# christoskokas/gtsam-vSLAM

Hardware: AMD Instinct MI355X
Metric: frames/sec (extract+match+localBA), 1500 feat stereo 752x480 (higher is better)
Workload: dtype u8/i32 (extract, match) + f64 (pose LM, local BA)

## Files before the change

### gtsam-vslam_amd/csrc/newpts.hip

```cpp
#include "proj_dev.hpp"
#include "track_dev.hpp"
#include "dmath.hpp"
#include <vector>
#include <mutex>

namespace vslam {

constexpr int NP_MAX_KF = 16;
constexpr int NP_MAX_ROWS = 4 * NP_MAX_KF;

struct NpKf {
    DPose Twc, Tcw;
    const vslam_keypoint* kpsL; const vslam_keypoint* kpsR;
    const uint8_t* descL; const uint8_t* descR;
    const int* rightIdxs; const int* leftIdxs; const int* unF; const int* unFR;
    int nL, nR;
    int skip;
};
struct NpArgs {
    NpKf kf[NP_MAX_KF];
    int nKf;
    const float* depth; const uint8_t* hasMp; const double* mpXyz; const uint8_t* mpDesc;
    double fx, fy, cx, cy, b; int w, h;
    float scalePyr[MAX_LEVELS], sigma[MAX_LEVELS];
// ... 55 lines not shown
            uint4* dd = (uint4*)(A.cdesc + (size_t)pos * 32);
            dd[0] = s[0]; dd[1] = s[1];
        }
        run += tot;
    }
    if (threadIdx.x == 0) A.count[0] = run < A.cap ? run : A.cap;
}

__global__ __launch_bounds__(256) void k_np_match(const NpArgs* __restrict__ tab) {
    const NpArgs& A = *lane_entry(tab, blockIdx.z);
    const int lane = threadIdx.x & 63;
    const int wave = __builtin_amdgcn_readfirstlane(threadIdx.x >> 6);
    const int c = blockIdx.x * 4 + wave, k = blockIdx.y + 1;
    if (k >= A.nKf || c >= A.count[0]) return;
    const NpKf& K = A.kf[k];
    int outL = -2, outR = -2;
    if (K.skip) { if (lane == 0) { A.match[((size_t)c * NP_MAX_KF + k) * 2] = -2; A.match[((size_t)c * NP_MAX_KF + k) * 2 + 1] = -2; } return; }
    const double wp[3] = {A.wPos[3 * (size_t)c], A.wPos[3 * (size_t)c + 1], A.wPos[3 * (size_t)c + 2]};
    double p[3];
    mat3_vec(K.Tcw.R, wp, p);
    for (int q = 0; q < 3; q++) p[q] += K.Tcw.t[q];
    const double pRx3 = p[0] - A.b;
    bool hasL = false, hasR = false;
    float pLx = 0, pLy = 0, pRx = 0, pRy = 0;
    if (!(p[2] <= 0.0)) {
        const double invZ = 1.0f / p[2];
        const double u = A.fx * p[0] * invZ + A.cx, v = A.fy * p[1] * invZ + A.cy;
        const double uR = A.fx * pRx3 * invZ + A.cx, vR = A.fy * p[1] * invZ + A.cy;
        if (!(u < 15 || v < 15 || u >= A.w - 15 || v >= A.h - 15)) { hasL = true; pLx = (float)u; pLy = (float)v; }
        if (!(uR < 15 || vR < 15 || uR >= A.w - 15 || vR >= A.h - 15)) { hasR = true; pRx = (float)uR; pRy = (float)vR; }
    }
    const double d[3] = {wp[0] - K.Twc.t[0], wp[1] - K.Twc.t[1], wp[2] - K.Twc.t[2]};
    const float dist = (float)sqrt(d[0] * d[0] + d[1] * d[1] + d[2] * d[2]);
    const float dif = A.mds[c] / dist;
    const double qs = log((double)dif) / (double)A.logScale;
    int predScale = (int)qs;
    predScale += (predScale < qs);
    if (predScale < 0) predScale = 0; else if (predScale >= A.nLev) predScale = A.nLev - 1;
    uint32_t md[8];
    {
        const uint32_t* pd = (const uint32_t*)(A.cdesc + (size_t)c * 32);
#pragma unroll
        for (int q = 0; q < 8; q++) md[q] = pd[q];
    }
    __shared__ ProjArgs sS[4];
    ProjArgs& S = sS[threadIdx.x >> 6];
    S.Mdev = nullptr; S.gate = nullptr; S.gateMin = 0; S.mpv = nullptr; S.M = 0; S.rightIdxs = nullptr; S.leftIdxs = nullptr;
    S.kps[0] = K.kpsL; S.kps[1] = K.kpsR; S.desc[0] = K.descL; S.desc[1] = K.descR; S.n[0] = K.nL; S.n[1] = K.nR;
    S.rad = 4.f;
    S.cellStart[0] = S.cellStart[1] = nullptr; S.cellIdx[0] = S.cellIdx[1] = nullptr;
#pragma unroll
    for (int l = 0; l < MAX_LEVELS; l++) S.scalePyr[l] = A.scalePyr[l];
    S.xMult = A.xMult; S.yMult = A.yMult; S.xGrids = A.xGrids; S.yGrids = A.yGrids; S.mode = PROJ_STEREO;
    unsigned long long l2[2] = {KEY_NONE, KEY_NONE}, r2[2] = {KEY_NONE, KEY_NONE};
    if (hasL && pLx > 0 && pLy > 0) scan_side<2>(S, 0, md, pLx, pLy, predScale, K.unF, l2);
    if (hasR && pRx > 0 && pRy > 0) scan_side<2>(S, 1, md, pRx, pRy, predScale, K.unFR, r2);
    if (lane == 0) {
        const int matchDistLBA = 50;
        const float ratioLBA = 0.6f;
        const unsigned long long POS = KEY_POS_MASK;
        int bestDist = 256, bestIdx = -1, bestLev = -1, bestLev2 = -1, secDist = 256;
        if (l2[0] != KEY_NONE && key_dist(l2[0]) < 256) { bestDist = key_dist(l2[0]); bestIdx = key_idx(l2[0]); bestLev = key_oct(l2[0]); }
        if (l2[1] != KEY_NONE && key_dist(l2[1]) < 256 && bestIdx >= 0) {
            secDist = key_dist(l2[1]);
            bestLev2 = ((l2[1] & POS) > (l2[0] & POS)) ? bestLev : key_oct(l2[1]);
        }
        int bestDistR = 256, bestIdxR = -1, bestLevR = -1, bestLevR2 = -1, secDistR = 256;
        if (r2[0] != KEY_NONE && key_dist(r2[0]) < 256) { bestDistR = key_dist(r2[0]); bestIdxR = key_idx(r2[0]); bestLevR = key_oct(r2[0]); }
        if (r2[1] != KEY_NONE && key_dist(r2[1]) < 256 && bestIdxR >= 0) { secDistR = key_dist(r2[1]); bestLevR2 = key_oct(r2[1]); }
        bool right = false;
        if (bestDist > bestDistR) { bestDist = bestDistR; secDist = secDistR; bestLev = bestLevR; bestLev2 = bestLevR2; right = true; }
        bool ok = !(bestDist > matchDistLBA);
        if (ok && bestLev == bestLev2 && (float)bestDist >= ratioLBA * (float)secDist) ok = false;
        if (ok) {
            const int keyL = A.key[2 * c], keyR = A.key[2 * c + 1];
            const NpKf& K0 = A.kf[0];
            const vslam_keypoint kk = right ? (keyR >= 0 ? K0.kpsR[keyR] : K0.kpsL[keyL]) : (keyL >= 0 ? K0.kpsL[keyL] : K0.kpsR[keyR]);
            const double dx = (double)(right ? pRx : pLx) - (double)kk.x, dy = (double)(right ? pRy : pLy) - (double)kk.y;
            if (!(sqrt(dx * dx + dy * dy) > 10.0)) ok = false;
        }
        if (ok) {
            if (right) { outR = bestIdxR; const int l = K.leftIdxs[bestIdxR]; outL = l >= 0 ? l : -1; }
            else { outL = bestIdx; const int r = K.rightIdxs[bestIdx]; outR = r >= 0 ? r : -1; }
        }
        A.match[((size_t)c * NP_MAX_KF + k) * 2] = outL;
        A.match[((size_t)c * NP_MAX_KF + k) * 2 + 1] = outR;
    }
}

__device__ __forceinline__ bool np_dlt_point(double* sA, int t, int rows, double* pt) {
    auto a = [&](int r, int q) -> double& { return sA[((size_t)(r * 4 + q)) * 64 + t]; };
    if (rows < 4) return false;
    double V[16];
#pragma unroll
    for (int i = 0; i < 16; i++) V[i] = (i % 5 == 0) ? 1.0 : 0.0;
    for (int sweep = 0; sweep < 30; sweep++) {
        bool rotated = false;
#pragma unroll
        for (int p = 0; p < 3; p++)
#pragma unroll
            for (int q = p + 1; q < 4; q++) {
                double alpha = 0, beta = 0, gamma = 0;
                for (int r = 0; r < rows; r++) {
                    const double ap = a(r, p), aq = a(r, q);
                    alpha += ap * ap; beta += aq * aq; gamma += ap * aq;
                }
                if (gamma == 0.0 || fabs(gamma) <= 1e-15 * sqrt(alpha * beta)) continue;
                rotated = true;
                const double zeta = (beta - alpha) / (2.0 * gamma);
// ... 743 lines not shown
```

### gtsam-vslam_amd/csrc/proj.hip

```cpp
#include "matcher.hpp"
#include "proj_dev.hpp"
#include "track_dev.hpp"

namespace vslam {

__device__ __forceinline__ void load_mp_desc(const vslam_mappoint_view* mp, uint32_t (&md)[8]) {
    const uint32_t* p = (const uint32_t*)mp->desc;
#pragma unroll
    for (int k = 0; k < 8; k++) md[k] = p[k];
}

constexpr int PROJ_CELLS_NT = 1024;
__device__ __forceinline__ void proj_cells_body(const ProjArgs& A, int side) {
    extern __shared__ int cellHist[];
    __shared__ int wsum[PROJ_CELLS_NT / 64];
    const int tid = threadIdx.x, lane = tid & 63, wave = tid >> 6;
    int* cs = A.cellStart[side];
    unsigned short* ci = A.cellIdx[side];
    if (!cs || !ci) return;
    const int nCells = A.xGrids * A.yGrids, n = A.n[side];
    const vslam_keypoint* kps = A.kps[side];
    for (int c = tid; c < nCells; c += PROJ_CELLS_NT) cellHist[c] = 0;
    __syncthreads();
    for (int idx = tid; idx < n; idx += PROJ_CELLS_NT) {
        int cx = __float2int_rn(kps[idx].x * A.xMult), cy = __float2int_rn(kps[idx].y * A.yMult);
        cx = cx < 0 ? 0 : (cx >= A.xGrids ? A.xGrids - 1 : cx);
        cy = cy < 0 ? 0 : (cy >= A.yGrids ? A.yGrids - 1 : cy);
        atomicAdd(&cellHist[cy * A.xGrids + cx], 1);
    }
    __syncthreads();
    const int per = (nCells + PROJ_CELLS_NT - 1) / PROJ_CELLS_NT;
    const int c0 = min(tid * per, nCells), c1 = min(c0 + per, nCells);
    int mine = 0;
    for (int c = c0; c < c1; c++) mine += cellHist[c];
    int incl = mine;
#pragma unroll
    for (int d = 1; d < 64; d <<= 1) { const int t = __shfl_up(incl, d); if (lane >= d) incl += t; }
    if (lane == 63) wsum[wave] = incl;
    __syncthreads();
    int run = incl - mine;
    for (int k = 0; k < wave; k++) run += wsum[k];
    for (int c = c0; c < c1; c++) { const int v = cellHist[c]; cs[c] = run; cellHist[c] = run; run += v; }
    if (tid == PROJ_CELLS_NT - 1) cs[nCells] = run;
    __syncthreads();
    for (int idx = tid; idx < n; idx += PROJ_CELLS_NT) {
        int cx = __float2int_rn(kps[idx].x * A.xMult), cy = __float2int_rn(kps[idx].y * A.yMult);
        cx = cx < 0 ? 0 : (cx >= A.xGrids ? A.xGrids - 1 : cx);
        cy = cy < 0 ? 0 : (cy >= A.yGrids ? A.yGrids - 1 : cy);
        ci[atomicAdd(&cellHist[cy * A.xGrids + cx], 1)] = (unsigned short)idx;
    }
}
__global__ __launch_bounds__(PROJ_CELLS_NT) void k_proj_cells(ProjArgs A) { proj_cells_body(A, blockIdx.x); }
__global__ __launch_bounds__(PROJ_CELLS_NT) void k_proj_cells_b(const ProjLane* __restrict__ lanes) {
    const ProjLane& L = *lane_entry(lanes, blockIdx.y);
    proj_cells_body(L.A, blockIdx.x);
}
void launch_proj_cells(hipStream_t s, const ProjArgs& A) {
    if (!A.cellStart[0]) return;
    hipLaunchKernelGGL(k_proj_cells, dim3(A.mode == PROJ_STEREO ? 2 : 1), dim3(PROJ_CELLS_NT), (size_t)PROJ_MAX_CELLS * sizeof(int), s, A);
}

__device__ __forceinline__ void proj_candidates_body(const ProjArgs& A, const int* __restrict__ matches,
                                                     unsigned long long* __restrict__ topk,
                                                     unsigned long long* __restrict__ stats) {
    const int lane = threadIdx.x & 63;
    const int wave = __builtin_amdgcn_readfirstlane(threadIdx.x >> 6);
    const int job = blockIdx.x * 4 + wave;
    __shared__ unsigned int sTests;
    if (A.gate && *A.gate < A.gateMin) return;
    int M = A.M;
    if (A.Mdev) M = min(M, *A.Mdev);
    if (threadIdx.x == 0) sTests = 0;
    __syncthreads();
    int tests = 0;
    if (job < 2 * M) {
        const int i = job >> 1, side = job & 1;
        unsigned long long out[PROJ_K];
#pragma unroll
        for (int j = 0; j < PROJ_K; j++) out[j] = KEY_NONE;
        const vslam_mappoint_view* mp = A.mpv + i;
        const bool skip = matches[2 * i] >= 0 || matches[2 * i + 1] >= 0;
        const bool inF = side ? (A.mode == PROJ_STEREO && mp->in_frame_r) : mp->in_frame;
        if (!skip && inF) {
            uint32_t md[8];
            load_mp_desc(mp, md);
            const float px = side ? mp->pred_rx : mp->pred_lx, py = side ? mp->pred_ry : mp->pred_ly;
            const int ps = side ? mp->scale_level_r : mp->scale_level_l;
            tests = scan_side<PROJ_K>(A, side, md, px, py, ps, nullptr, out);
        }
        if (lane < PROJ_K) {
            unsigned long long v = out[0];
#pragma unroll
            for (int j = 1; j < PROJ_K; j++) v = lane == j ? out[j] : v;
            topk[(size_t)job * PROJ_K + lane] = v;
        }
    }
    if (lane == 0 && tests) atomicAdd(&sTests, (unsigned int)tests);
    __syncthreads();
    if (threadIdx.x == 0 && sTests) atomicAdd(&stats[3], (unsigned long long)sTests);
}

__global__ __launch_bounds__(256) void k_proj_candidates(ProjArgs A, const int* __restrict__ matches, unsigned long long* __restrict__ topk,
                                                         unsigned long long* __restrict__ stats) {
    proj_candidates_body(A, matches, topk, stats);
}
__global__ __launch_bounds__(256) void k_proj_candidates_b(const ProjLane* __restrict__ lanes) {
    const ProjLane& L = *lane_entry(lanes, blockIdx.y);
    if ((int)(blockIdx.x * 4) >= 2 * L.A.M) return;
    proj_candidates_body(L.A, L.matches, L.topk, L.stats);
}

void launch_proj_candidates(hipStream_t s, const ProjArgs& A, const int* matches,
                            unsigned long long* topk, unsigned long long* stats) {
    if (A.M <= 0) return;
    hipLaunchKernelGGL(k_proj_candidates, dim3((2 * A.M + 3) / 4), dim3(256), 0, s, A, matches, topk, stats);
}

__device__ __forceinline__ int proj_decide(unsigned long long l1, unsigned long long l2, unsigned long long r1,
                                           unsigned long long r2, int mode) {
    const int matchDistProj = 100;
    const float ratioProj = 0.8f;
    int bestDist = 256, bestIdx = -1, bestLev = -1, bestLev2 = -1, secDist = 256;
    if (l1 != KEY_NONE) { bestDist = key_dist(l1); bestIdx = key_idx(l1); bestLev = key_oct(l1); }
    if (l2 != KEY_NONE) { secDist = key_dist(l2); bestLev2 = key_oct(l2); }
    int bestDistR = 256, bestIdxR = -1, bestLevR = -1, bestLevR2 = -1, secDistR = 256;
    if (r1 != KEY_NONE) { bestDistR = key_dist(r1); bestIdxR = key_idx(r1); bestLevR = key_oct(r1); }
    if (r2 != KEY_NONE) { secDistR = key_dist(r2); bestLevR2 = key_oct(r2); }
    if (bestDist >= 256) { bestDist = 256; bestIdx = -1; bestLev = -1; }
    if (secDist >= 256) { secDist = 256; bestLev2 = -1; }
    if (bestDistR >= 256) { bestDistR = 256; bestIdxR = -1; bestLevR = -1; }
    if (secDistR >= 256) { secDistR = 256; bestLevR2 = -1; }
    bool right = false;
    if (bestDist > bestDistR) {
        bestDist = bestDistR; secDist = secDistR; bestLev = bestLevR; bestLev2 = bestLevR2; bestIdx = bestIdxR;
        right = true;
    }
    if (mode == PROJ_MONO) {
        if (bestDist > matchDistProj + 50) return -1;
        if (bestLev == bestLev2 && (double)bestDist >= ((double)ratioProj + 0.1) * (double)secDist) return -1;
        return bestIdx;
    }
    if (bestDist > matchDistProj) return -1;
    if (bestLev == bestLev2 && (float)bestDist >= ratioProj * (float)secDist) return -1;
    return (right ? 1 << 16 : 0) | bestIdx;
}

constexpr int PROJ_SUPER = 512;
constexpr int PROJ_NT = 512;
constexpr int PROJ_PAR_PASSES = 8;
constexpr int PROJ_PAR_ROUNDS = 16;

__device__ __forceinline__ void lds_order() { asm volatile("s_waitcnt lgkmcnt(0)" ::: "memory"); }

__device__ __forceinline__ void proj_resolve_body(const ProjArgs& A, const unsigned long long* __restrict__ topk,
                                                  int* __restrict__ matchedL, int* __restrict__ matchedR,
                                                  int* __restrict__ matches, int* __restrict__ outp, int forceSeq, int superN) {
    extern __shared__ int claims[];
    int* cl = claims;
    int* cr = claims + A.n[0];
    int* ri = cr + A.n[1];
    int* li = ri + A.n[0];
    int* tl = li + A.n[1];
    int* tr = tl + A.n[0];
    int* spair = tr + A.n[1];
    unsigned long long* skeys = (unsigned long long*)(((uintptr_t)(spair + 2 * superN) + 15) & ~(uintptr_t)15);
    const int tid = threadIdx.x, lane = tid & 63, wave = tid >> 6;
    if (A.gate && *A.gate < A.gateMin) return;
    int M = A.M;
    if (A.Mdev) M = min(M, *A.Mdev);
    for (int k = tid; k < A.n[0]; k += PROJ_NT) { cl[k] = matchedL[k]; ri[k] = A.mode == PROJ_STEREO ? A.rightIdxs[k] : -1; tl[k] = INT_MAX; }
    for (int k = tid; k < A.n[1]; k += PROJ_NT) { cr[k] = matchedR[k]; li[k] = A.leftIdxs[k]; tr[k] = INT_MAX; }
    int nMatches = 0;
    static_assert(PROJ_K == 8, "lane layout assumes 8 keys per side");
    const int q = lane >> 2, e = lane & 3, side = e >> 1, half = e & 1;

    __shared__ int sChanged, sFall, sCount;
    bool solved = false;
    const int Mtot = M;
    int roundsUsed = -1;
    if (!forceSeq && Mtot > 0 && Mtot <= PROJ_PAR_PASSES * (PROJ_NT / 4)) {
        int* decT = (int*)skeys;
        unsigned long long K[PROJ_PAR_PASSES][4];
        int PV[PROJ_PAR_PASSES];
#pragma unroll
        for (int p = 0; p < PROJ_PAR_PASSES; p++) {
            const int i = p * (PROJ_NT / 4) + wave * 16 + q;
            K[p][0] = K[p][1] = K[p][2] = K[p][3] = KEY_NONE;
            PV[p] = 0;
            if (i < Mtot) {
                const ulonglong2* src = (const ulonglong2*)(topk + (size_t)i * 16 + e * 4);
                const ulonglong2 a = src[0], b2v = src[1];
                K[p][0] = a.x; K[p][1] = a.y; K[p][2] = b2v.x; K[p][3] = b2v.y;
                PV[p] = matches[2 * (size_t)i + (e & 1)];
            }
        }
        for (int i = tid; i < Mtot; i += PROJ_NT) decT[i] = -1;
        if (tid == 0) { sFall = 0; sCount = 0; }
        __syncthreads();
        for (int round = 0; round < PROJ_PAR_ROUNDS; round++) {
            if (tid == 0) sChanged = 0;
            for (int i = tid; i < Mtot; i += PROJ_NT) {
                const int d = decT[i];
                if (d < 0) continue;
                const int idx = d & 0xffff;
                int cL, cR;
                if (d >> 16) { cR = idx; cL = li[idx]; } else { cL = idx; cR = ri[idx]; }
                if (cL >= 0) atomicMin(&tl[cL], i);
                if (cR >= 0) atomicMin(&tr[cR], i);
            }
// ... 115 lines not shown
            if (dec >= 0) {
                const int idx = dec & 0xffff;
                if (dec >> 16) { cRq = idx; cLq = li[idx]; } else { cLq = idx; cRq = ri[idx]; }
            }
            if (e == 0 && dec >= 0) {
                if (cLq >= 0) atomicMin(&tl[cLq], q);
                if (cRq >= 0) atomicMin(&tr[cRq], q);
            }
            lds_order();
            if (!skip) {
                const int* tt = side ? tr : tl;
#pragma unroll
                for (int j = 0; j < 4; j++)
                    if (k4[j] != KEY_NONE && tt[key_idx(k4[j])] < q) bad = true;
                if ((cLq >= 0 && tl[cLq] < q) || (cRq >= 0 && tr[cRq] < q)) bad = true;
            }
            lds_order();
            if (e == 0 && dec >= 0) {
                if (cLq >= 0) tl[cLq] = INT_MAX;
                if (cRq >= 0) tr[cRq] = INT_MAX;
            }
            if (__ballot(bad) == 0ull) {
                if (e == 0 && dec >= 0) {
                    const int i = sc + pl;
                    if (cLq >= 0) { cl[cLq] = i; matches[2 * (size_t)i] = cLq; }
                    if (cRq >= 0) { cr[cRq] = i; matches[2 * (size_t)i + 1] = cRq; }
                }
                nMatches += __popcll(__ballot(e == 0 && dec >= 0));
                lds_order();
                continue;
            }
            for (int qq = 0; qq < 16; qq++) {
                const int pli = base + qq;
                if (pli >= n) break;
                const int i = sc + pli;
                if (__shfl((int)skip, qq * 4)) continue;
                const int sd = lane >= PROJ_K ? 1 : 0;
                unsigned long long key = KEY_NONE;
                if (lane < 16) key = skeys[(size_t)pli * 16 + lane];
                const bool valid = key != KEY_NONE;
                bool fre = false;
                if (valid) fre = (sd ? cr[key_idx(key)] : cl[key_idx(key)]) < 0;
                const unsigned long long vmask = __ballot(valid), fmask = __ballot(fre);
                unsigned long long b1k[2], b2k[2];
#pragma unroll
                for (int s = 0; s < 2; s++) {
                    const int sh = s * PROJ_K;
                    const unsigned vmm = (unsigned)((vmask >> sh) & 0xffu);
                    unsigned fmm = (unsigned)((fmask >> sh) & 0xffu);
                    if (vmm == 0xffu && __popc(fmm) < 2) {
                        const vslam_mappoint_view* mp = A.mpv + i;
                        uint32_t md[8];
                        load_mp_desc(mp, md);
                        unsigned long long o2k[2] = {KEY_NONE, KEY_NONE};
                        const float px = s ? mp->pred_rx : mp->pred_lx, py = s ? mp->pred_ry : mp->pred_ly;
                        const int ps = s ? mp->scale_level_r : mp->scale_level_l;
                        scan_side<2>(A, s, md, px, py, ps, s ? cr : cl, o2k);
                        b1k[s] = o2k[0];
                        b2k[s] = o2k[1];
                    } else {
                        int l1 = -1, l2 = -1;
                        if (fmm) { l1 = __ffs(fmm) - 1; fmm &= fmm - 1; }
                        if (fmm) { l2 = __ffs(fmm) - 1; }
                        const unsigned long long k1 = __shfl(key, (l1 < 0 ? 0 : l1) + sh);
                        const unsigned long long k2 = __shfl(key, (l2 < 0 ? 0 : l2) + sh);
                        b1k[s] = l1 < 0 ? KEY_NONE : k1;
                        b2k[s] = l2 < 0 ? KEY_NONE : k2;
                    }
                }
                const int d2 = proj_decide(b1k[0], b2k[0], b1k[1], b2k[1], A.mode);
                if (d2 < 0) continue;
                nMatches++;
                if (lane == 0) {
                    const int idx = d2 & 0xffff;
                    if (d2 >> 16) {
                        cr[idx] = i;
                        matches[2 * (size_t)i + 1] = idx;
                        const int l = li[idx];
                        if (l >= 0) { matches[2 * (size_t)i] = l; cl[l] = i; }
                    } else {
                        cl[idx] = i;
                        matches[2 * (size_t)i] = idx;
                        const int r = ri[idx];
                        if (r >= 0) { matches[2 * (size_t)i + 1] = r; cr[r] = i; }
                    }
                }
                lds_order();
            }
        }
    }
    __syncthreads();
    for (int k = tid; k < A.n[0]; k += PROJ_NT) matchedL[k] = cl[k];
    for (int k = tid; k < A.n[1]; k += PROJ_NT) matchedR[k] = cr[k];
    if (tid == 0) { outp[0] = nMatches; outp[1] = roundsUsed; }
}

__global__ __launch_bounds__(PROJ_NT) void k_proj_resolve(ProjArgs A, const unsigned long long* __restrict__ topk, int* __restrict__ matchedL,
                                                     int* __restrict__ matchedR, int* __restrict__ matches, int* __restrict__ outp, int forceSeq, int superN) {
    proj_resolve_body(A, topk, matchedL, matchedR, matches, outp, forceSeq, superN);
}
__global__ __launch_bounds__(PROJ_NT) void k_proj_resolve_b(const ProjLane* __restrict__ lanes, int forceSeq, int superN) {
    const ProjLane& L = *lane_entry(lanes, blockIdx.x);
    proj_resolve_body(L.A, L.topk, L.matchedL, L.matchedR, L.matches, L.out, forceSeq, superN);
}

static size_t proj_resolve_lds(int nL, int nR, int superN) {
    return (size_t)(3 * (nL + nR) + 2 * superN) * sizeof(int) + 32 + (size_t)superN * 16 * sizeof(unsigned long long);
}
constexpr size_t PROJ_LDS_CAP = 159 * 1024;
static int proj_super(int nL, int nR) {
    int sp = PROJ_SUPER;
    while (sp > 32 && proj_resolve_lds(nL, nR, sp) > PROJ_LDS_CAP) sp /= 2;
    return sp;
}
static void proj_attrs() {
    static bool attr = false;
    if (attr) return;
    (void)hipFuncSetAttribute((const void*)k_proj_resolve, hipFuncAttributeMaxDynamicSharedMemorySize, (int)PROJ_LDS_CAP);
    (void)hipFuncSetAttribute((const void*)k_proj_resolve_b, hipFuncAttributeMaxDynamicSharedMemorySize, (int)PROJ_LDS_CAP);
    attr = true;
}

void launch_proj_batch(hipStream_t s, const ProjLane* dLanes, int B, int maxM, int maxL, int maxR, StageTimer* tm, bool buildCells) {
    if (B <= 0 || maxM <= 0) return;
    proj_attrs();
    const int forceSeq = getenv("VSLAM_PROJ_SEQUENTIAL") ? 1 : 0;
    int t = -1;
    if (buildCells) {
        t = tm ? tm->begin("proj_cells") : -1;
        hipLaunchKernelGGL(k_proj_cells_b, dim3(2, B), dim3(PROJ_CELLS_NT), (size_t)PROJ_MAX_CELLS * sizeof(int), s, dLanes);
        if (tm) tm->end(t);
    }
    t = tm ? tm->begin("proj_candidates") : -1;
    hipLaunchKernelGGL(k_proj_candidates_b, dim3((2 * maxM + 3) / 4, B), dim3(256), 0, s, dLanes);
    if (tm) { tm->end(t); t = tm->begin("proj_resolve"); }
    const int sp = proj_super(maxL, maxR);
    hipLaunchKernelGGL(k_proj_resolve_b, dim3(B), dim3(PROJ_NT), proj_resolve_lds(maxL, maxR, sp), s, dLanes, forceSeq, sp);
    if (tm) tm->end(t);
}

void launch_proj_resolve(hipStream_t s, const ProjArgs& A, const unsigned long long* topk, int* matchedL, int* matchedR,
                         int* matches, int* out) {
    const int sp = proj_super(A.n[0], A.n[1]);
    const size_t sh = proj_resolve_lds(A.n[0], A.n[1], sp);
    proj_attrs();
    const int forceSeq = getenv("VSLAM_PROJ_SEQUENTIAL") ? 1 : 0;
    hipLaunchKernelGGL(k_proj_resolve, dim3(1), dim3(PROJ_NT), sh, s, A, topk, matchedL, matchedR, matches, out, forceSeq, sp);
#ifdef VSLAM_PROJ_STAMPS
    { int o[2]; (void)hipStreamSynchronize(s); (void)hipMemcpy(o, out, sizeof(o), hipMemcpyDeviceToHost); fprintf(stderr, "proj_resolve: matches %d, fixed-point rounds %d (-1 = sequential walk)\n", o[0], o[1]); }
#endif
}

}

using namespace vslam;

vslam_status vslam_matcher::ensure_proj_cap(int M) {
    if (M <= projCap && d_matchedL && d_projOut) return VSLAM_OK;
    if (M > projCap) {
        hipFree(d_mpv); hipFree(d_topk); hipFree(d_matches);
        projCap = vslam::align_up(std::max(M, 1), 1024);
        VS_HIP(hipMalloc(&d_mpv, (size_t)projCap * sizeof(vslam_mappoint_view)));
        VS_HIP(hipMalloc(&d_topk, (size_t)projCap * 2 * PROJ_K * sizeof(unsigned long long)));
        VS_HIP(hipMalloc(&d_matches, (size_t)projCap * 2 * sizeof(int)));
    }
    if (!d_projOut) VS_HIP(hipMalloc(&d_projOut, 4 * sizeof(int)));
    if (!d_matchedL) {
        VS_HIP(hipMalloc(&d_matchedL, (size_t)65536 * sizeof(int)));
        VS_HIP(hipMalloc(&d_matchedR, (size_t)65536 * sizeof(int)));
    }
    for (int s = 0; s < 2; s++) {
        if (!d_cellStart[s]) VS_HIP(hipMalloc(&d_cellStart[s], (size_t)(PROJ_MAX_CELLS + 1) * sizeof(int)));
        if (!d_cellIdx[s]) VS_HIP(hipMalloc(&d_cellIdx[s], (size_t)65536 * sizeof(unsigned short)));
    }
    return VSLAM_OK;
}

void vslam_matcher::proj_lane(vslam::ProjLane& L, int M, float rad, const int* Mdev, const int* gate, int gateMin, int mode) {
    ProjArgs& A = L.A;
    A = ProjArgs{};
    A.Mdev = Mdev; A.gate = gate; A.gateMin = gateMin; A.mode = mode;
    for (int s = 0; s < 2; s++) { A.kps[s] = d_kps[s]; A.desc[s] = d_desc[s]; A.n[s] = nKeys[s]; }
    A.mpv = d_mpv; A.M = M; A.rad = rad;
    for (int l = 0; l < feL->nLevels; l++) A.scalePyr[l] = feL->scalePyramid[l];
    const float imageRatio = (float)rig.width / (float)rig.height;
    A.xGrids = 64;
    A.yGrids = cv_ceil_f((float)A.xGrids / imageRatio);
    A.xMult = (float)A.xGrids / (float)rig.width;
    A.yMult = (float)A.yGrids / (float)rig.height;
    A.rightIdxs = d_rightIdxs; A.leftIdxs = d_leftIdxs;
    if (A.xGrids * A.yGrids <= PROJ_MAX_CELLS)
        for (int s = 0; s < 2; s++) { A.cellStart[s] = d_cellStart[s]; A.cellIdx[s] = d_cellIdx[s]; }
    L.matches = d_matches; L.topk = d_topk; L.stats = d_stats; L.matchedL = d_matchedL; L.matchedR = d_matchedR; L.out = d_projOut;
}

vslam_status vslam_matcher::proj_enqueue(int M, float rad, const int* Mdev, const int* gate, int gateMin, int mode) {
    ProjLane L;
    proj_lane(L, M, rad, Mdev, gate, gateMin, mode);
    const ProjArgs& A = L.A;
    int t = timer.begin("proj_cells");
    launch_proj_cells(stream, A);
    timer.end(t);
    t = timer.begin("proj_candidates");
    launch_proj_candidates(stream, A, d_matches, d_topk, d_stats);
    timer.end(t);
    t = timer.begin("proj_resolve");
    launch_proj_resolve(stream, A, d_topk, d_matchedL, d_matchedR, d_matches, d_projOut);
    timer.end(t);
// ... 111 lines not shown
    if (nMatches) for (int t = 0; t < nTargets; t++) nMatches[t] = 0;
    for (size_t k = 0; k < (size_t)nLast * nTargets; k++) matchOut[k] = -1;
    if (nLast == 0 || nTargets == 0) return VSLAM_OK;
    VS_HIP(hipSetDevice(device));
    size_t at = 0;
    auto put = [&](size_t bytes) { const size_t a = at; at = (at + bytes + 255) & ~(size_t)255; return a; };
    const size_t oLanes = put((size_t)nTargets * sizeof(ProjLane)), oMpv = put((size_t)nLast * sizeof(vslam_mappoint_view));
    const size_t oTab = put((size_t)nMatched * sizeof(int)), oOut = put((size_t)nTargets * 4 * sizeof(int)), oStats = put(4 * sizeof(unsigned long long));
    const size_t oMt = put((size_t)nTargets * nLast * 2 * sizeof(int));
    const size_t oTopk = put((size_t)nTargets * nLast * 2 * PROJ_K * sizeof(unsigned long long));
    const size_t oCs = put((size_t)nTargets * (PROJ_MAX_CELLS + 1) * sizeof(int));
    std::vector<size_t> oCi(nTargets);
    for (int t = 0; t < nTargets; t++) oCi[t] = put((size_t)std::max(nTarget[t], 1) * sizeof(unsigned short));
    if (at > winCap) {
        VS_HIP(hipStreamSynchronize(stream));
        hipFree(d_win); d_win = nullptr; winCap = 0;
        VS_HIP(hipMalloc((void**)&d_win, at));
        winCap = at;
    }
    uint8_t* w = d_win;
    vslam_mappoint_view* mpv = (vslam_mappoint_view*)(w + oMpv);
    int* tab = (int*)(w + oTab);
    std::vector<ProjLane> lanes(nTargets);
    const KeyBlockLayout ol = key_block_layout(nLast, 0);
    for (int t = 0; t < nTargets; t++) {
        ProjLane& L = lanes[t];
        proj_lane(L, nLast, rad, nullptr, nullptr, 0, PROJ_RADIUS);
        ProjArgs& A = L.A;
        const KeyBlockLayout o = key_block_layout(nTarget[t], 0);
        const uint8_t* blk = (const uint8_t*)targetKeys[t];
        A.kps[0] = nTarget[t] ? (const vslam_keypoint*)(blk + o.kpsL) : nullptr; A.desc[0] = nTarget[t] ? blk + o.descL : nullptr; A.n[0] = nTarget[t];
        A.kps[1] = nullptr; A.desc[1] = nullptr; A.n[1] = 0;
        A.mpv = mpv; A.rightIdxs = nullptr; A.leftIdxs = nullptr;
        const bool bucketed = A.xGrids * A.yGrids <= PROJ_MAX_CELLS;
        A.cellStart[0] = bucketed ? (int*)(w + oCs) + (size_t)t * (PROJ_MAX_CELLS + 1) : nullptr;
        A.cellIdx[0] = bucketed ? (unsigned short*)(w + oCi[t]) : nullptr;
        A.cellStart[1] = nullptr; A.cellIdx[1] = nullptr;
        L.matches = (int*)(w + oMt) + (size_t)t * nLast * 2;
        L.topk = (unsigned long long*)(w + oTopk) + (size_t)t * nLast * 2 * PROJ_K;
        L.stats = (unsigned long long*)(w + oStats);
        L.matchedL = tab; L.matchedR = tab; L.out = (int*)(w + oOut) + 4 * t;
    }
    VS_HIP(hipMemcpyAsync(w + oLanes, lanes.data(), (size_t)nTargets * sizeof(ProjLane), hipMemcpyHostToDevice, stream));
    VS_HIP(hipMemcpyAsync(tab, matchedL, (size_t)nMatched * sizeof(int), hipMemcpyHostToDevice, stream));
    VS_HIP(hipMemsetAsync(w + oMt, 0xff, (size_t)nTargets * nLast * 2 * sizeof(int), stream));
    VS_HIP(hipMemsetAsync(w + oStats, 0, 4 * sizeof(unsigned long long), stream));
    VS_HIP(hipMemsetAsync(w + oOut, 0, (size_t)nTargets * 4 * sizeof(int), stream));
    const uint8_t* lb = (const uint8_t*)lastKeys;
    hipLaunchKernelGGL(k_radius_views, dim3((nLast + 255) / 256), dim3(256), 0, stream, (const vslam_keypoint*)(lb + ol.kpsL), lb + ol.descL, nLast, mpv);
    const ProjLane* dLanes = (const ProjLane*)(w + oLanes);
    proj_attrs();
    if (lanes[0].A.cellStart[0])
        hipLaunchKernelGGL(k_proj_cells_b, dim3(1, nTargets), dim3(PROJ_CELLS_NT), (size_t)PROJ_MAX_CELLS * sizeof(int), stream, dLanes);
    hipLaunchKernelGGL(k_proj_candidates_b, dim3((2 * nLast + 3) / 4, nTargets), dim3(256), 0, stream, dLanes);
    for (int t = 0; t < nTargets; t++)
        launch_proj_resolve(stream, lanes[t].A, lanes[t].topk, tab, tab, lanes[t].matches, lanes[t].out);
    VS_HIP(hipGetLastError());
    std::vector<int> mt((size_t)nTargets * nLast * 2), outs((size_t)nTargets * 4);
    VS_HIP(hipMemcpyAsync(mt.data(), w + oMt, mt.size() * sizeof(int), hipMemcpyDeviceToHost, stream));
    VS_HIP(hipMemcpyAsync(outs.data(), w + oOut, outs.size() * sizeof(int), hipMemcpyDeviceToHost, stream));
    VS_HIP(hipMemcpyAsync(matchedL, tab, (size_t)nMatched * sizeof(int), hipMemcpyDeviceToHost, stream));
    VS_HIP(hipStreamSynchronize(stream));
    for (int t = 0; t < nTargets; t++) {
        for (int i = 0; i < nLast; i++) matchOut[(size_t)t * nLast + i] = mt[((size_t)t * nLast + i) * 2];
        if (nMatches) nMatches[t] = outs[4 * (size_t)t];
    }
    return VSLAM_OK;
}

extern "C" vslam_status vslam_match_by_radius_window(vslam_matcher* m, const void* last_keys, int32_t n_last,
                                                     const void* const* target_keys, const int32_t* n_target, int32_t n_targets,
                                                     float rad, int32_t* matched_idxs_l, int32_t n_matched,
                                                     int32_t* match_out, int32_t* n_matches) {
    if (!m) return VSLAM_ERR_INVALID;
    return m->match_radius_window(last_keys, n_last, target_keys, n_target, n_targets, rad, matched_idxs_l, n_matched, match_out, n_matches);
}
```

### gtsam-vslam_amd/csrc/proj_dev.hpp

```cpp
#pragma once
#include "matcher.hpp"

namespace vslam {

__device__ __forceinline__ int p_cvFloor(float v) { int i = (int)v; return i - (i > v); }
__device__ __forceinline__ int p_cvCeil(float v) { int i = (int)v; return i + (i < v); }

constexpr unsigned long long KEY_NONE = ~0ull;
__device__ __forceinline__ unsigned long long make_key(int dist, int cell, int idx, int oct) {
    return ((unsigned long long)dist << KEY_DIST_SHIFT) | ((unsigned long long)cell << KEY_CELL_SHIFT) |
           ((unsigned long long)idx << KEY_IDX_SHIFT) | (unsigned long long)(oct & ((1 << KEY_OCT_BITS) - 1));
}
__device__ __forceinline__ int key_dist(unsigned long long k) { return (int)(k >> KEY_DIST_SHIFT); }
__device__ __forceinline__ int key_idx(unsigned long long k) { return (int)((k >> KEY_IDX_SHIFT) & ((1 << KEY_IDX_BITS) - 1)); }
__device__ __forceinline__ int key_oct(unsigned long long k) { return (int)(k & ((1 << KEY_OCT_BITS) - 1)); }
constexpr unsigned long long KEY_POS_MASK = ((1ull << KEY_DIST_SHIFT) - 1ull) & ~((1ull << KEY_IDX_SHIFT) - 1ull);

template <int K>
__device__ __forceinline__ void insert_sorted(unsigned long long (&a)[K], unsigned long long key) {
#pragma unroll
    for (int j = 0; j < K; j++) {
        if (key < a[j]) { const unsigned long long t = a[j]; a[j] = key; key = t; }
    }
}

__device__ __forceinline__ unsigned long long wave_min_u64(unsigned long long v) {
#pragma unroll
    for (int d = 32; d >= 1; d >>= 1) {
        const unsigned long long o = __shfl_xor(v, d);
        v = o < v ? o : v;
    }
    return v;
}

template <int K>
__device__ int scan_side(const ProjArgs& A, int side, const uint32_t (&md)[8], float px, float py,
                         int predScale, const int* claimed, unsigned long long (&out)[K]) {
    const int lane = threadIdx.x & 63;
    unsigned long long top[K];
#pragma unroll
    for (int j = 0; j < K; j++) top[j] = KEY_NONE;
    int tests = 0;
    const float radius = A.scalePyr[predScale] * A.rad;
    const int minX = max(0, p_cvFloor((px - radius) * A.xMult));
    const int maxX = min(A.xGrids - 1, p_cvCeil((px + radius) * A.xMult));
    const int minY = max(0, p_cvFloor((py - radius) * A.yMult));
    const int maxY = min(A.yGrids - 1, p_cvCeil((py + radius) * A.yMult));
    const bool any = !(minX >= A.xGrids || minY >= A.yGrids || maxX < 0 || maxY < 0);
    const vslam_keypoint* kps = A.kps[side];
    const uint8_t* desc = A.desc[side];
    auto consider = [&](int idx) {
        const float kx = kps[idx].x, ky = kps[idx].y;
        int cx = __float2int_rn(kx * A.xMult), cy = __float2int_rn(ky * A.yMult);
        cx = cx < 0 ? 0 : (cx >= A.xGrids ? A.xGrids - 1 : cx);
        cy = cy < 0 ? 0 : (cy >= A.yGrids ? A.yGrids - 1 : cy);
        if (cx < minX || cx > maxX || cy < minY || cy > maxY) return;
        const int oct = kps[idx].octave;
        if (oct > predScale + 1 || oct < predScale - 1) return;
        if (!(fabsf(kx - px) < radius && fabsf(ky - py) < radius)) return;
        if (claimed && claimed[idx] >= 0) return;
        if (A.mode == PROJ_RADIUS) {
            const double dx = (double)kx - (double)px, dy = (double)ky - (double)py;
            if (!(sqrt(dx * dx + dy * dy) > 10.0)) return;
        }
        const uint4* pr = (const uint4*)(desc + (size_t)idx * 32);
        const uint4 r0 = pr[0], r1 = pr[1];
        const int dist = __popc(md[0] ^ r0.x) + __popc(md[1] ^ r0.y) + __popc(md[2] ^ r0.z) +
                         __popc(md[3] ^ r0.w) + __popc(md[4] ^ r1.x) + __popc(md[5] ^ r1.y) +
                         __popc(md[6] ^ r1.z) + __popc(md[7] ^ r1.w);
        tests++;
        insert_sorted<K>(top, make_key(dist, cy * A.xGrids + cx, idx, oct));
    };
    const int nrows = maxY - minY + 1;
    if (any && A.cellStart[side] && nrows <= 64) {
        const int* cs = A.cellStart[side];
        const unsigned short* ci = A.cellIdx[side];
        int rbeg = 0, rlen = 0;
        if (lane < nrows) {
            const int c0 = (minY + lane) * A.xGrids;
            rbeg = cs[c0 + minX];
            rlen = cs[c0 + maxX + 1] - rbeg;
        }
        int incl = rlen;
#pragma unroll
        for (int d = 1; d < 64; d <<= 1) { const int t = __shfl_up(incl, d); if (lane >= d) incl += t; }
        const int total = __shfl(incl, 63);
        for (int base = 0; base < total; base += 64) {
            const int p = base + lane;
            int r = 0;
            for (int q = 0; q < nrows; q++) r += (p >= __shfl(incl, q));
            r = r < nrows ? r : nrows - 1;
            const int re = __shfl(incl, r), rl = __shfl(rlen, r), rb = __shfl(rbeg, r);
            if (p < total) consider((int)ci[rb + (p - (re - rl))]);
        }
    } else if (any) {
        const int n = A.n[side];
        for (int idx = lane; idx < n; idx += 64) consider(idx);
    }
#pragma unroll
    for (int r = 0; r < K; r++) {
        const unsigned long long head = top[0];
        const unsigned long long m = wave_min_u64(head);
        out[r] = m;
        if (head == m && m != KEY_NONE) {
#pragma unroll
            for (int j = 0; j + 1 < K; j++) top[j] = top[j + 1];
            top[K - 1] = KEY_NONE;
        }
    }
#pragma unroll
    for (int d = 32; d >= 1; d >>= 1) tests += __shfl_xor(tests, d);
    return tests;
}


}
```

Measured before the change: 29770.

## Add sparse single-pass rank-select path for projection candidate scan

When a map point's search window holds at most 64 keypoints, scan_side now gives each lane one candidate and picks the top-K by computing ranks with ballot/readlane instead of per-lane sorted insertion and repeated wave min reductions. Results are returned as one per-lane selected key instead of a K-array, and callers read back entries with readlane. It also replaces the per-row prefix-sum and search with a simple readlane walk. An env var turns the path off, and an optional histogram debug build is added. The rank loop costs O(valid candidates) readlanes per wave, which may cost more than the old path when windows are dense.

```diff
diff --git a/gtsam-vslam_amd/csrc/newpts.hip b/gtsam-vslam_amd/csrc/newpts.hip
--- a/gtsam-vslam_amd/csrc/newpts.hip
+++ b/gtsam-vslam_amd/csrc/newpts.hip
@@ -131,9 +131,11 @@
 #pragma unroll
     for (int l = 0; l < MAX_LEVELS; l++) S.scalePyr[l] = A.scalePyr[l];
     S.xMult = A.xMult; S.yMult = A.yMult; S.xGrids = A.xGrids; S.yGrids = A.yGrids; S.mode = PROJ_STEREO;
-    unsigned long long l2[2] = {KEY_NONE, KEY_NONE}, r2[2] = {KEY_NONE, KEY_NONE};
-    if (hasL && pLx > 0 && pLy > 0) scan_side<2>(S, 0, md, pLx, pLy, predScale, K.unF, l2);
-    if (hasR && pRx > 0 && pRy > 0) scan_side<2>(S, 1, md, pRx, pRy, predScale, K.unFR, r2);
+    unsigned long long lsel = KEY_NONE, rsel = KEY_NONE;
+    if (hasL && pLx > 0 && pLy > 0) scan_side<2>(S, 0, md, pLx, pLy, predScale, K.unF, lsel);
+    if (hasR && pRx > 0 && pRy > 0) scan_side<2>(S, 1, md, pRx, pRy, predScale, K.unFR, rsel);
+    const unsigned long long l2[2] = {wave_read_u64(lsel, 0), wave_read_u64(lsel, 1)};
+    const unsigned long long r2[2] = {wave_read_u64(rsel, 0), wave_read_u64(rsel, 1)};
     if (lane == 0) {
         const int matchDistLBA = 50;
         const float ratioLBA = 0.6f;
diff --git a/gtsam-vslam_amd/csrc/proj.hip b/gtsam-vslam_amd/csrc/proj.hip
--- a/gtsam-vslam_amd/csrc/proj.hip
+++ b/gtsam-vslam_amd/csrc/proj.hip
@@ -62,7 +62,7 @@
 
 __device__ __forceinline__ void proj_candidates_body(const ProjArgs& A, const int* __restrict__ matches,
                                                      unsigned long long* __restrict__ topk,
-                                                     unsigned long long* __restrict__ stats) {
+                                                     unsigned long long* __restrict__ stats, int sparse) {
     const int lane = threadIdx.x & 63;
     const int wave = __builtin_amdgcn_readfirstlane(threadIdx.x >> 6);
     const int job = blockIdx.x * 4 + wave;
@@ -75,9 +75,7 @@
     int tests = 0;
     if (job < 2 * M) {
         const int i = job >> 1, side = job & 1;
-        unsigned long long out[PROJ_K];
-#pragma unroll
-        for (int j = 0; j < PROJ_K; j++) out[j] = KEY_NONE;
+        unsigned long long sel = KEY_NONE;
         const vslam_mappoint_view* mp = A.mpv + i;
         const bool skip = matches[2 * i] >= 0 || matches[2 * i + 1] >= 0;
         const bool inF = side ? (A.mode == PROJ_STEREO && mp->in_frame_r) : mp->in_frame;
@@ -86,14 +84,15 @@
             load_mp_desc(mp, md);
             const float px = side ? mp->pred_rx : mp->pred_lx, py = side ? mp->pred_ry : mp->pred_ly;
             const int ps = side ? mp->scale_level_r : mp->scale_level_l;
-            tests = scan_side<PROJ_K>(A, side, md, px, py, ps, nullptr, out);
+#ifdef VSLAM_PROJ_HIST
+            int visited = 0;
+            tests = scan_side<PROJ_K>(A, side, md, px, py, ps, nullptr, sel, sparse != 0, &visited);
+            proj_hist_add(visited, tests);
+#else
+            tests = scan_side<PROJ_K>(A, side, md, px, py, ps, nullptr, sel, sparse != 0);
+#endif
         }
-        if (lane < PROJ_K) {
-            unsigned long long v = out[0];
-#pragma unroll
-            for (int j = 1; j < PROJ_K; j++) v = lane == j ? out[j] : v;
-            topk[(size_t)job * PROJ_K + lane] = v;
-        }
+        if (lane < PROJ_K) topk[(size_t)job * PROJ_K + lane] = sel;
     }
     if (lane == 0 && tests) atomicAdd(&sTests, (unsigned int)tests);
     __syncthreads();
@@ -101,19 +100,26 @@
 }
 
 __global__ __launch_bounds__(256) void k_proj_candidates(ProjArgs A, const int* __restrict__ matches, unsigned long long* __restrict__ topk,
-                                                         unsigned long long* __restrict__ stats) {
-    proj_candidates_body(A, matches, topk, stats);
-}
-__global__ __launch_bounds__(256) void k_proj_candidates_b(const ProjLane* __restrict__ lanes) {
+                                                         unsigned long long* __restrict__ stats, int sparse) {
+    proj_candidates_body(A, matches, topk, stats, sparse);
+}
+__global__ __launch_bounds__(256) void k_proj_candidates_b(const ProjLane* __restrict__ lanes, int sparse) {
     const ProjLane& L = *lane_entry(lanes, blockIdx.y);
     if ((int)(blockIdx.x * 4) >= 2 * L.A.M) return;
-    proj_candidates_body(L.A, L.matches, L.topk, L.stats);
-}
+    proj_candidates_body(L.A, L.matches, L.topk, L.stats, sparse);
+}
+
+static int proj_select() {
+    const char* e = getenv("VSLAM_PROJ_SELECT");
+    return (e && e[0] == '0') ? 0 : 1;
+}
+
+static int proj_resolve_flags() { return (getenv("VSLAM_PROJ_SEQUENTIAL") ? 1 : 0) | (proj_select() << 1); }
 
 void launch_proj_candidates(hipStream_t s, const ProjArgs& A, const int* matches,
                             unsigned long long* topk, unsigned long long* stats) {
     if (A.M <= 0) return;
-    hipLaunchKernelGGL(k_proj_candidates, dim3((2 * A.M + 3) / 4), dim3(256), 0, s, A, matches, topk, stats);
+    hipLaunchKernelGGL(k_proj_candidates, dim3((2 * A.M + 3) / 4), dim3(256), 0, s, A, matches, topk, stats, proj_select());
 }
 
 __device__ __forceinline__ int proj_decide(unsigned long long l1, unsigned long long l2, unsigned long long r1,
@@ -154,7 +160,8 @@
 
 __device__ __forceinline__ void proj_resolve_body(const ProjArgs& A, const unsigned long long* __restrict__ topk,
                                                   int* __restrict__ matchedL, int* __restrict__ matchedR,
-                                                  int* __restrict__ matches, int* __restrict__ outp, int forceSeq, int superN) {
+                                                  int* __restrict__ matches, int* __restrict__ outp, int flags, int superN) {
+    const int forceSeq = flags & 1, sparse = (flags >> 1) & 1;
     extern __shared__ int claims[];
     int* cl = claims;
     int* cr = claims + A.n[0];
@@ -376,12 +383,12 @@
                         const vslam_mappoint_view* mp = A.mpv + i;
                         uint32_t md[8];
                         load_mp_desc(mp, md);
-                        unsigned long long o2k[2] = {KEY_NONE, KEY_NONE};
+                        unsigned long long o2k = KEY_NONE;
                         const float px = s ? mp->pred_rx : mp->pred_lx, py = s ? mp->pred_ry : mp->pred_ly;
                         const int ps = s ? mp->scale_level_r : mp->scale_level_l;
-                        scan_side<2>(A, s, md, px, py, ps, s ? cr : cl, o2k);
-                        b1k[s] = o2k[0];
-                        b2k[s] = o2k[1];
+                        scan_side<2>(A, s, md, px, py, ps, s ? cr : cl, o2k, sparse != 0);
+                        b1k[s] = wave_read_u64(o2k, 0);
+                        b2k[s] = wave_read_u64(o2k, 1);
                     } else {
                         int l1 = -1, l2 = -1;
                         if (fmm) { l1 = __ffs(fmm) - 1; fmm &= fmm - 1; }
@@ -420,12 +427,12 @@
 }
 
 __global__ __launch_bounds__(PROJ_NT) void k_proj_resolve(ProjArgs A, const unsigned long long* __restrict__ topk, int* __restrict__ matchedL,
-                                                     int* __restrict__ matchedR, int* __restrict__ matches, int* __restrict__ outp, int forceSeq, int superN) {
-    proj_resolve_body(A, topk, matchedL, matchedR, matches, outp, forceSeq, superN);
-}
-__global__ __launch_bounds__(PROJ_NT) void k_proj_resolve_b(const ProjLane* __restrict__ lanes, int forceSeq, int superN) {
+                                                     int* __restrict__ matchedR, int* __restrict__ matches, int* __restrict__ outp, int flags, int superN) {
+    proj_resolve_body(A, topk, matchedL, matchedR, matches, outp, flags, superN);
+}
+__global__ __launch_bounds__(PROJ_NT) void k_proj_resolve_b(const ProjLane* __restrict__ lanes, int flags, int superN) {
     const ProjLane& L = *lane_entry(lanes, blockIdx.x);
-    proj_resolve_body(L.A, L.topk, L.matchedL, L.matchedR, L.matches, L.out, forceSeq, superN);
+    proj_resolve_body(L.A, L.topk, L.matchedL, L.matchedR, L.matches, L.out, flags, superN);
 }
 
 static size_t proj_resolve_lds(int nL, int nR, int superN) {
@@ -448,7 +455,7 @@
 void launch_proj_batch(hipStream_t s, const ProjLane* dLanes, int B, int maxM, int maxL, int maxR, StageTimer* tm, bool buildCells) {
     if (B <= 0 || maxM <= 0) return;
     proj_attrs();
-    const int forceSeq = getenv("VSLAM_PROJ_SEQUENTIAL") ? 1 : 0;
+    const int sparse = proj_select();
     int t = -1;
     if (buildCells) {
         t = tm ? tm->begin("proj_cells") : -1;
@@ -456,10 +463,10 @@
         if (tm) tm->end(t);
     }
     t = tm ? tm->begin("proj_candidates") : -1;
-    hipLaunchKernelGGL(k_proj_candidates_b, dim3((2 * maxM + 3) / 4, B), dim3(256), 0, s, dLanes);
+    hipLaunchKernelGGL(k_proj_candidates_b, dim3((2 * maxM + 3) / 4, B), dim3(256), 0, s, dLanes, sparse);
     if (tm) { tm->end(t); t = tm->begin("proj_resolve"); }
     const int sp = proj_super(maxL, maxR);
-    hipLaunchKernelGGL(k_proj_resolve_b, dim3(B), dim3(PROJ_NT), proj_resolve_lds(maxL, maxR, sp), s, dLanes, forceSeq, sp);
+    hipLaunchKernelGGL(k_proj_resolve_b, dim3(B), dim3(PROJ_NT), proj_resolve_lds(maxL, maxR, sp), s, dLanes, proj_resolve_flags(), sp);
     if (tm) tm->end(t);
 }
 
@@ -468,8 +475,7 @@
     const int sp = proj_super(A.n[0], A.n[1]);
     const size_t sh = proj_resolve_lds(A.n[0], A.n[1], sp);
     proj_attrs();
-    const int forceSeq = getenv("VSLAM_PROJ_SEQUENTIAL") ? 1 : 0;
-    hipLaunchKernelGGL(k_proj_resolve, dim3(1), dim3(PROJ_NT), sh, s, A, topk, matchedL, matchedR, matches, out, forceSeq, sp);
+    hipLaunchKernelGGL(k_proj_resolve, dim3(1), dim3(PROJ_NT), sh, s, A, topk, matchedL, matchedR, matches, out, proj_resolve_flags(), sp);
 #ifdef VSLAM_PROJ_STAMPS
     { int o[2]; (void)hipStreamSynchronize(s); (void)hipMemcpy(o, out, sizeof(o), hipMemcpyDeviceToHost); fprintf(stderr, "proj_resolve: matches %d, fixed-point rounds %d (-1 = sequential walk)\n", o[0], o[1]); }
 #endif
@@ -478,6 +484,15 @@
 }
 
 using namespace vslam;
+
+#ifdef VSLAM_PROJ_HIST
+extern "C" vslam_status vslam_debug_proj_hist(unsigned long long* out) {
+    if (!out) return VSLAM_ERR_INVALID;
+    VS_HIP(hipDeviceSynchronize());
+    VS_HIP(hipMemcpyFromSymbol(out, HIP_SYMBOL(g_projHist), sizeof(unsigned long long) * 2 * 66));
+    return VSLAM_OK;
+}
+#endif
 
 vslam_status vslam_matcher::ensure_proj_cap(int M) {
     if (M <= projCap && d_matchedL && d_projOut) return VSLAM_OK;
@@ -695,7 +710,7 @@
     proj_attrs();
     if (lanes[0].A.cellStart[0])
         hipLaunchKernelGGL(k_proj_cells_b, dim3(1, nTargets), dim3(PROJ_CELLS_NT), (size_t)PROJ_MAX_CELLS * sizeof(int), stream, dLanes);
-    hipLaunchKernelGGL(k_proj_candidates_b, dim3((2 * nLast + 3) / 4, nTargets), dim3(256), 0, stream, dLanes);
+    hipLaunchKernelGGL(k_proj_candidates_b, dim3((2 * nLast + 3) / 4, nTargets), dim3(256), 0, stream, dLanes, proj_select());
     for (int t = 0; t < nTargets; t++)
         launch_proj_resolve(stream, lanes[t].A, lanes[t].topk, tab, tab, lanes[t].matches, lanes[t].out);
     VS_HIP(hipGetLastError());
diff --git a/gtsam-vslam_amd/csrc/proj_dev.hpp b/gtsam-vslam_amd/csrc/proj_dev.hpp
--- a/gtsam-vslam_amd/csrc/proj_dev.hpp
+++ b/gtsam-vslam_amd/csrc/proj_dev.hpp
@@ -33,14 +33,49 @@
     return v;
 }
 
+__device__ __forceinline__ unsigned long long wave_read_u64(unsigned long long v, int src) {
+    const unsigned lo = (unsigned)__builtin_amdgcn_readlane((int)(unsigned)v, src);
+    const unsigned hi = (unsigned)__builtin_amdgcn_readlane((int)(unsigned)(v >> 32), src);
+    return ((unsigned long long)hi << 32) | lo;
+}
+
+template <int K>
+__device__ __forceinline__ unsigned long long sel_from_array(const unsigned long long (&out)[K], int lane) {
+    unsigned long long v = KEY_NONE;
+#pragma unroll
+    for (int j = 0; j < K; j++) v = lane == j ? out[j] : v;
+    return v;
+}
+
+template <int K>
+__device__ __forceinline__ unsigned long long rank_select(unsigned long long key, int lane) {
+    const bool valid = key != KEY_NONE;
+    int rank = 0;
+    for (unsigned long long m = __ballot(valid); m; m &= m - 1) rank += wave_read_u64(key, __builtin_ctzll(m)) < key;
+    unsigned long long res = KEY_NONE;
+    for (unsigned long long m = __ballot(valid && rank < K); m; m &= m - 1) {
+        const int b = __builtin_ctzll(m);
+        const int rb = __builtin_amdgcn_readlane(rank, b);
+        const unsigned long long kb = wave_read_u64(key, b);
+        res = lane == rb ? kb : res;
+    }
+    return res;
+}
+
+#ifdef VSLAM_PROJ_HIST
+static __device__ unsigned long long g_projHist[2][66];
+__device__ __forceinline__ void proj_hist_add(int visited, int tests) {
+    if ((threadIdx.x & 63) != 0) return;
+    atomicAdd(&g_projHist[0][min(visited, 65)], 1ull);
+    atomicAdd(&g_projHist[1][min(tests, 65)], 1ull);
+}
+#endif
+
 template <int K>
 __device__ int scan_side(const ProjArgs& A, int side, const uint32_t (&md)[8], float px, float py,
-                         int predScale, const int* claimed, unsigned long long (&out)[K]) {
+                         int predScale, const int* claimed, unsigned long long& sel, bool sparse = true, int* visited = nullptr) {
     const int lane = threadIdx.x & 63;
-    unsigned long long top[K];
-#pragma unroll
-    for (int j = 0; j < K; j++) top[j] = KEY_NONE;
-    int tests = 0;
+    sel = KEY_NONE;
     const float radius = A.scalePyr[predScale] * A.rad;
     const int minX = max(0, p_cvFloor((px - radius) * A.xMult));
     const int maxX = min(A.xGrids - 1, p_cvCeil((px + radius) * A.xMult));
@@ -49,65 +84,101 @@
     const bool any = !(minX >= A.xGrids || minY >= A.yGrids || maxX < 0 || maxY < 0);
     const vslam_keypoint* kps = A.kps[side];
     const uint8_t* desc = A.desc[side];
-    auto consider = [&](int idx) {
+    auto consider = [&](int idx) -> unsigned long long {
         const float kx = kps[idx].x, ky = kps[idx].y;
         int cx = __float2int_rn(kx * A.xMult), cy = __float2int_rn(ky * A.yMult);
         cx = cx < 0 ? 0 : (cx >= A.xGrids ? A.xGrids - 1 : cx);
         cy = cy < 0 ? 0 : (cy >= A.yGrids ? A.yGrids - 1 : cy);
-        if (cx < minX || cx > maxX || cy < minY || cy > maxY) return;
+        if (cx < minX || cx > maxX || cy < minY || cy > maxY) return KEY_NONE;
         const int oct = kps[idx].octave;
-        if (oct > predScale + 1 || oct < predScale - 1) return;
-        if (!(fabsf(kx - px) < radius && fabsf(ky - py) < radius)) return;
-        if (claimed && claimed[idx] >= 0) return;
+        if (oct > predScale + 1 || oct < predScale - 1) return KEY_NONE;
+        if (!(fabsf(kx - px) < radius && fabsf(ky - py) < radius)) return KEY_NONE;
+        if (claimed && claimed[idx] >= 0) return KEY_NONE;
         if (A.mode == PROJ_RADIUS) {
             const double dx = (double)kx - (double)px, dy = (double)ky - (double)py;
-            if (!(sqrt(dx * dx + dy * dy) > 10.0)) return;
+            if (!(sqrt(dx * dx + dy * dy) > 10.0)) return KEY_NONE;
         }
         const uint4* pr = (const uint4*)(desc + (size_t)idx * 32);
         const uint4 r0 = pr[0], r1 = pr[1];
         const int dist = __popc(md[0] ^ r0.x) + __popc(md[1] ^ r0.y) + __popc(md[2] ^ r0.z) +
                          __popc(md[3] ^ r0.w) + __popc(md[4] ^ r1.x) + __popc(md[5] ^ r1.y) +
                          __popc(md[6] ^ r1.z) + __popc(md[7] ^ r1.w);
-        tests++;
-        insert_sorted<K>(top, make_key(dist, cy * A.xGrids + cx, idx, oct));
+        return make_key(dist, cy * A.xGrids + cx, idx, oct);
     };
-    const int nrows = maxY - minY + 1;
-    if (any && A.cellStart[side] && nrows <= 64) {
+    if (!any) return 0;
+    const int nrows = __builtin_amdgcn_readfirstlane(maxY - minY + 1);
+    const bool bucketed = A.cellStart[side] && nrows <= 64;
+    int rbeg = 0, rlen = 0;
+    if (bucketed) {
         const int* cs = A.cellStart[side];
         const unsigned short* ci = A.cellIdx[side];
-        int rbeg = 0, rlen = 0;
         if (lane < nrows) {
             const int c0 = (minY + lane) * A.xGrids;
             rbeg = cs[c0 + minX];
             rlen = cs[c0 + maxX + 1] - rbeg;
         }
+        if (sparse) {
+            int total = 0, src = -1;
+            for (int q = 0; q < nrows; q++) {
+                const int lq = __builtin_amdgcn_readlane(rlen, q), bq = __builtin_amdgcn_readlane(rbeg, q);
+                const int o = lane - total;
+                if ((unsigned)o < (unsigned)lq) src = bq + o;
+                total += lq;
+            }
+            if (total <= 64) {
+                unsigned long long key = KEY_NONE;
+                if (src >= 0) key = consider((int)ci[src]);
+                sel = rank_select<K>(key, lane);
+                if (visited) *visited = total;
+                return __popcll(__ballot(key != KEY_NONE));
+            }
+        }
+    }
+    unsigned long long top[K];
+#pragma unroll
+    for (int j = 0; j < K; j++) top[j] = KEY_NONE;
+    int tests = 0;
+    auto take = [&](unsigned long long key) {
+        if (key == KEY_NONE) return;
+        tests++;
+        insert_sorted<K>(top, key);
+    };
+    if (bucketed) {
+        const unsigned short* ci = A.cellIdx[side];
         int incl = rlen;
 #pragma unroll
         for (int d = 1; d < 64; d <<= 1) { const int t = __shfl_up(incl, d); if (lane >= d) incl += t; }
         const int total = __shfl(incl, 63);
+        if (visited) *visited = total;
         for (int base = 0; base < total; base += 64) {
             const int p = base + lane;
             int r = 0;
             for (int q = 0; q < nrows; q++) r += (p >= __shfl(incl, q));
             r = r < nrows ? r : nrows - 1;
             const int re = __shfl(incl, r), rl = __shfl(rlen, r), rb = __shfl(rbeg, r);
-            if (p < total) consider((int)ci[rb + (p - (re - rl))]);
+            if (p < total) take(consider((int)ci[rb + (p - (re - rl))]));
         }
-    } else if (any) {
+    } else {
         const int n = A.n[side];
-        for (int idx = lane; idx < n; idx += 64) consider(idx);
+        if (visited) *visited = n;
+        for (int idx = lane; idx < n; idx += 64) take(consider(idx));
     }
+    unsigned long long out[K];
+#pragma unroll
+    for (int j = 0; j < K; j++) out[j] = KEY_NONE;
 #pragma unroll
     for (int r = 0; r < K; r++) {
         const unsigned long long head = top[0];
         const unsigned long long m = wave_min_u64(head);
+        if (m == KEY_NONE) break;
         out[r] = m;
-        if (head == m && m != KEY_NONE) {
+        if (head == m) {
 #pragma unroll
             for (int j = 0; j + 1 < K; j++) top[j] = top[j + 1];
             top[K - 1] = KEY_NONE;
         }
     }
+    sel = sel_from_array<K>(out, lane);
 #pragma unroll
     for (int d = 32; d >= 1; d >>= 1) tests += __shfl_xor(tests, d);
     return tests;
```

Result: faster. 30380 (median of 6 runs) (+2.1%).
